# dv66/Distributed-Active-Learning

Measured on AMD Instinct MI355X. Metric: pool rows scored/sec (density-weighted uncertainty), 1–8 GPU; % MFMA/HBM peak, higher is better.
Workload: dtype f32 (fp16-split MFMA, fp32 accumulate); 1 GPU; config4: U[0,1) 2,000,000 x 256 fp32 pool (default_rng(0)), T=10 depth-4 forest, entropy x density, k=100, E={0..9}; pool_rows=2000000, features=256, trees=10, k=100, parallelism=single GPU

## Files before the change

### distributed-active-learning_amd/csrc/gram_csym_body.inc

```
  constexpr int HV = C::HALVES;
  __shared__ __attribute__((aligned(16))) float4 lds[2 * C::F4];
  __shared__ typename C::racc_t rowacc[HV * kSB];
  __shared__ int claim_lds[2];

  const int tid = threadIdx.x;
  const int wave = __builtin_amdgcn_readfirstlane(tid >> 6), lane = tid & 63;
  const int half = wave / C::WPS, wave4 = wave % C::WPS;
  if constexpr (C::WAVES == 8 && DAL_GRAM_PRIO8 != 0) {
    if (DAL_GRAM_PRIO8 > 0 ? wave >= 4 : wave < 4) __builtin_amdgcn_s_setprio(1);
  }
  const int li = lane & 15, lq = lane >> 4;
  const int G = gridDim.x, g = blockIdx.x;
  for (int e = tid; e < HV * kSB; e += C::NT) rowacc[e] = 0.0;

  const GramSchedule<HV> sched(srow0, n_srb, j_lo, j_hi, skip_lo, skip_hi, ns_active, chunk_j, n_chunks, contig, G,
                               g);

  constexpr int RPP = 64 / C::SLOTS;
  static_assert((RPP & (RPP - 1)) == 0 && (C::PIECES & (C::PIECES - 1)) == 0, "row parts must occupy disjoint bits");
  const unsigned rowbytes = static_cast<unsigned>(ldh * 2);
  const unsigned dst0 = __builtin_amdgcn_readfirstlane(
      static_cast<unsigned>(reinterpret_cast<uintptr_t>((AS3 float4*)(lds + wave * C::PIECES * 64))));
  auto issue = [&](int buf, int J, int h, int slice) {
    J = __builtin_amdgcn_readfirstlane(J);
    slice = __builtin_amdgcn_readfirstlane(slice);
    const char* sbase = reinterpret_cast<const char*>(
        ucols + (static_cast<int64_t>(J - jcol0) * 256 + h * C::SC) * ldh + slice_off + C::sub_off(slice));
    const unsigned fl = fresh_lane();
    const unsigned lrow = fl / C::SLOTS + static_cast<unsigned>(wave * C::PIECES * RPP);
    const unsigned vlane = lrow * rowbytes + (((fl % C::SLOTS) ^ static_cast<unsigned>(C::swz(lrow))) << 4);
#pragma unroll
    for (int q = 0; q < C::PIECES; ++q) {
      const unsigned dst = dst0 + static_cast<unsigned>(buf * C::STAGE + q * 1024);
      const unsigned voff = (vlane ^ (static_cast<unsigned>(C::swz(q * RPP)) << 4)) +
                            static_cast<unsigned>(q * RPP) * rowbytes;
      lds_dma_x4(voff, dst, sbase);
    }
  };

  f16x8 ah[C::RT][C::NKS];
  auto load_a = [&](int ru, int slice) {
    const int P = sched.rowP(ru, half);
    if (HV > 1 && !sched.live(P)) return;
    const uint16_t* pb = urows + static_cast<int64_t>(P - srow0) * kSB * ldh + slice_off + C::sub_off(slice);
    const unsigned fl = fresh_lane();
    const unsigned lrow = static_cast<unsigned>((wave4 * C::RPW + (fl & 15)) * ldh + (fl >> 4) * 8);
    const unsigned tstep = static_cast<unsigned>(16 * ldh);
#pragma unroll
    for (int rt = 0; rt < C::RT; ++rt)
#pragma unroll
      for (int c = 0; c < C::NKS; ++c)
        ah[rt][c] = __builtin_nontemporal_load(reinterpret_cast<const f16x8*>(pb + lrow + rt * tstep + c * C::LG * 8));
  };
  const int b_base = li * C::SLOTS + (lq ^ (C::swz(li) & 3));
  const int b_swz = C::swz(li) & ~3;
  auto b_off = [&](int c) { return b_base + ((c * C::LG) ^ b_swz); };

  typename C::acc4 mc[C::NCH][C::RT];
  [[maybe_unused]] const int mx_scale = kFp4ScaleWord;
  f16x8 bh[2];
  auto compute = [&](int buf, bool fresh_stage, int ct0 = 0, int ct1 = C::NCT) {
    auto load_b = [&](int set, int c, int ct) {
      bh[set] = __builtin_bit_cast(f16x8, lds[buf * C::F4 + ct * 16 * C::SLOTS + b_off(c)]);
    };
    if (ct0 == 0) load_b(0, 0, 0);
#pragma unroll
    for (int ct = ct0; ct < ct1; ++ct) {
      __builtin_amdgcn_sched_barrier(0);
      const bool fresh = fresh_stage && ct == 0;
#pragma unroll
      for (int c = 0; c < C::NKS; ++c) {
        constexpr int KPC = C::NKS / C::NCH;
        const int ch = c / KPC;
        const int i = ct * C::NKS + c, cur = i & 1;
        if (c + 1 < C::NKS)
          load_b(cur ^ 1, c + 1, ct);
        else if (ct + 1 < C::NCT)
          load_b(cur ^ 1, 0, ct + 1);
        const typename C::acc4 zero = {};
#pragma unroll
        for (int rt = 0; rt < C::RT; ++rt)
          mc[ch][rt] = C::mfma(bh[cur], ah[rt][c], (c % KPC == 0 && fresh) ? zero : mc[ch][rt], mx_scale);
      }
      constexpr int NM = C::RT;
#pragma unroll
      for (int c = 0; c < C::NKS; ++c) {
        __builtin_amdgcn_sched_group_barrier(0x100, 1, 0);
        __builtin_amdgcn_sched_group_barrier(0x008, NM, 0);
      }
      __builtin_amdgcn_sched_barrier(0);
    }
  };
  auto fold_rows = [&]() {
#pragma unroll
    for (int ch = 0; ch < C::NCH; ++ch)
#pragma unroll
      for (int t0 = 0; t0 < C::RT; t0 += 8) {
        typename C::sum_t x[8];
#pragma unroll
        for (int rt = 0; rt < 8; ++rt) {
          const typename C::acc4 m = mc[ch][t0 + rt];
          x[rt] = C::lane_sum(m);
        }
#pragma unroll
        for (int k = 0; k < 4; ++k) x[k] = swap_add<true>(x[k], x[k + 4]);
#pragma unroll
        for (int k = 0; k < 2; ++k) x[k] = swap_add<false>(x[k], x[k + 2]);
        const int row = wave * C::RPW + (t0 + 2 * (lq & 1) + 4 * (lq >> 1)) * 16 + li;
        C::row_add(&rowacc[row], x[0]);
        C::row_add(&rowacc[row + 16], x[1]);
      }
  };
  auto flush_one = [&](typename C::racc_t& slot, int64_t out_row) {
    const typename C::racc_t v = slot;
    if (v != 0) atomicAdd(acc_out + out_row, static_cast<unsigned long long>(static_cast<long long>(v)));
    slot = 0;
  };
  auto flush_rows = [&](int ru) {
    for (int e = tid; e < HV * kSB; e += C::NT) {
      const int P = sched.rowP(ru, e / kSB);
      if (sched.live(P)) flush_one(rowacc[e], static_cast<int64_t>(P) * kSB + e % kSB);
    }
  };
  auto block_sync = [&]() {
    asm volatile("s_waitcnt vmcnt(0) lgkmcnt(0)" ::: "memory");
    __syncthreads();
  };
  auto stage_sync = [&]() { block_sync(); };

  GramClaimCursor<HV> cur(sched, n_slices * C::NSUB);
  const bool dyn = claim_slot >= 0;
  int claim_par = 0;
  auto claim_begin = [&]() {
    if (dyn && tid == 0)
      claim_lds[claim_par] =
          G + static_cast<int>(__hip_atomic_fetch_add(&g_claim[claim_slot].next, 1u, __ATOMIC_RELAXED,
                                                      __HIP_MEMORY_SCOPE_AGENT));
  };
  auto claim_end = [&](int last) {
    const int u = dyn ? __builtin_amdgcn_readfirstlane(claim_lds[claim_par]) : cur.static_next(last);
    claim_par ^= 1;
    return u;
  };
  auto claim_take = [&]() {
    while (!cur.claimed(claim_end(cur.v_next))) {
      claim_begin();
      if (dyn) block_sync();
    }
  };
  auto leave = [&]() {
    if (dyn && tid == 0) {
      const unsigned before =
          __hip_atomic_fetch_add(&g_claim[claim_slot].done, 1u, __ATOMIC_RELAXED, __HIP_MEMORY_SCOPE_AGENT);
      if (before + 1 == static_cast<unsigned>(G)) {
        __hip_atomic_store(&g_claim[claim_slot].next, 0u, __ATOMIC_RELAXED, __HIP_MEMORY_SCOPE_AGENT);
        __hip_atomic_store(&g_claim[claim_slot].done, 0u, __ATOMIC_RELAXED, __HIP_MEMORY_SCOPE_AGENT);
      }
    }
  };
  if (!cur.claimed(cur.first_unit())) {
    claim_begin();
    if (dyn) block_sync();
    claim_take();
  }
  if (!cur.start()) {
    leave();
    return;
  }
  issue(0, cur.J, 0, cur.slice);
  load_a(cur.ru, cur.slice);
  claim_begin();
  int buf = 0;
  int flushRU = -1;

  while (true) {
    const bool act = cur.acts(half);

#pragma unroll
    for (int s = 0; s < C::SPP; ++s) {
      stage_sync();
      if constexpr (C::WIDE && DAL_GRAM_STAGGER > 0) {
        if (flushRU >= 0) {
          flush_rows(flushRU);
          flushRU = -1;
        }
        auto look_ahead = [&]() {
          if (cur.new_unit) claim_take();
          cur.peek();
          if (cur.has_next) issue(buf ^ 1, cur.next_J, 0, cur.next_slice());
        };
        const bool lead = lookahead_tiles(wave, C::WAVES, DAL_GRAM_STAGGER) == 0;
        if (!act) {
          look_ahead();
        } else {
          if (lead) look_ahead();
          compute(buf, true, 0, DAL_GRAM_STAGGER);
          if (!lead) look_ahead();
          compute(buf, true, DAL_GRAM_STAGGER, C::NCT);
          fold_rows();
        }
        buf ^= 1;
        continue;
      }
      if (s == 0) {
        if (cur.new_unit) claim_take();
        cur.peek();
        if (flushRU >= 0) {
          flush_rows(flushRU);
          flushRU = -1;
        }
      }
      if (s + 1 < C::SPP) {
        issue(buf ^ 1, cur.J, s + 1, cur.slice);
      } else if (cur.has_next) {
        issue(buf ^ 1, cur.next_J, 0, cur.next_slice());
      }
      if (act) {
        compute(buf, s % C::SPF == 0);
        if (s % C::SPF == C::SPF - 1) fold_rows();
      }
      buf ^= 1;
    }

    if (cur.rows_change) flushRU = cur.ru;
    if (!cur.has_next) break;
    if (cur.advance()) load_a(cur.ru, cur.slice);
    if (cur.new_unit) claim_begin();
  }
  block_sync();
  if (flushRU >= 0) flush_rows(flushRU);
  leave();
```

### distributed-active-learning_amd/csrc/gram_fp4.hpp

```cpp
#pragma once

#include "gram_i8.hpp"

#ifdef __HIPCC__
#define DAL_FP4_HD __host__ __device__
#else
#define DAL_FP4_HD
#endif

namespace dal {

constexpr float kFp4Step = 32.0f;
constexpr int kFp4AccShift = 18;
constexpr int kFp4Max = 12;
constexpr int kFp4ChainMax = 16 * 256 * kFp4Max * kFp4Max;
constexpr int kFp4RowMax = 256 * 256 * kFp4Max * kFp4Max;
static_assert(kFp4Step == kI8Step && kFp4AccShift == kI8AccShift, "the unit of G is the int8 form's");
static_assert(kFp4ChainMax == 589824 && 4 * kFp4ChainMax < (1 << 24),
              "fp32 chains and a lane's four columns are exact");
static_assert(kFp4RowMax == 9437184 && kFp4RowMax < (1LL << 31), "int32 row sums");

DAL_FP4_HD inline int quant_fp4(float h) {
  const float m = __builtin_fabsf(h) * (1.0f / kFp4Step);
  const int g = m > 10.0f ? 12 : m > 7.0f ? 8 : m > 5.0f ? 6 : m > 3.5f ? 4 : m > 2.5f ? 3 : m > 1.5f ? 2
                 : m > 0.5f ? 1 : 0;
  return h < 0.0f ? -g : g;
}

DAL_FP4_HD inline unsigned code_fp4(int g) {
  const unsigned m = static_cast<unsigned>(g < 0 ? -g : g);
  const unsigned idx = m <= 4u ? m : m == 6u ? 5u : m == 8u ? 6u : 7u;
  return idx | (g < 0 ? 8u : 0u);
}
DAL_FP4_HD inline int decode_fp4(unsigned code) {
  const unsigned idx = code & 7u;
  const int m = static_cast<int>(idx <= 4u ? idx : idx == 5u ? 6u : idx == 6u ? 8u : 12u);
  return code & 8u ? -m : m;
}

DAL_FP4_HD inline void requant_fp4(double& h, double& l) {
  const double hq = static_cast<double>(kFp4Step) * quant_fp4(static_cast<float>(h));
  l = (h - hq) + l;
  h = hq;
}

}
```

### distributed-active-learning_amd/csrc/gram_i8.hpp

```cpp
#pragma once

#ifdef __HIPCC__
#define DAL_I8_HD __host__ __device__
#else
#define DAL_I8_HD
#endif

namespace dal {

constexpr float kI8Step = 32.0f;
constexpr int kI8AccShift = 18;

DAL_I8_HD inline int quant_i8(float h) {
  const float q = __builtin_rintf(h * (1.0f / kI8Step));
  return static_cast<int>(q > 127.0f ? 127.0f : q >= -127.0f ? q : -127.0f);
}

DAL_I8_HD inline void requant_i8(double& h, double& l) {
  const double hq = static_cast<double>(kI8Step) * quant_i8(static_cast<float>(h));
  l = (h - hq) + l;
  h = hq;
}

}
```

### distributed-active-learning_amd/csrc/gram_schedule.hpp

```cpp
#pragma once

#include <stdint.h>

#include <utility>
#include <vector>

#if defined(__HIPCC__)
#define DAL_HD __host__ __device__ __forceinline__
#else
#define DAL_HD inline
#endif

namespace dal {

template <class I>
DAL_HD bool sb_takes(I P, I Q) {
  return Q == P || (Q > P && ((P + Q) & 1) == 0) || (Q < P && ((P + Q) & 1));
}

template <int HV>
struct GramSchedule {
  static_assert(HV == 1 || HV == 2 || HV == 4, "one, two or four super blocks per row unit");
  static constexpr bool form_ok(int contig) { return HV == 1 || !contig; }

  int srow0, n_srb, j_lo, j_hi, skip_lo, skip_hi, ns_active, chunk_j, n_chunks, contig, G, g;
  int n_ru;
  int sk_lo, skl;
  int nje;
  int nre;
  int64_t ka, kb;
  int n_seg;

  DAL_HD GramSchedule(int srow0_, int n_srb_, int j_lo_, int j_hi_, int skip_lo_, int skip_hi_, int ns_active_,
                      int chunk_j_, int n_chunks_, int contig_, int G_ = 1, int g_ = 0)
      : srow0(srow0_), n_srb(n_srb_), j_lo(j_lo_), j_hi(j_hi_), skip_lo(skip_lo_), skip_hi(skip_hi_),
        ns_active(ns_active_), chunk_j(chunk_j_), n_chunks(n_chunks_), contig(contig_), G(G_), g(g_) {
    n_ru = HV == 1 ? n_srb : 2 * ((n_srb + 2 * HV - 1) / (2 * HV));
    sk_lo = skip_lo > j_lo ? skip_lo : j_lo;
    const int sk_hi = skip_hi < j_hi ? skip_hi : j_hi;
    skl = contig && sk_hi > sk_lo ? sk_hi - sk_lo : 0;
    nje = j_hi - j_lo - skl;
    const int nre0 = ns_active - srow0;
    nre = nre0 < n_srb ? (nre0 > 0 ? nre0 : 0) : n_srb;
    ka = raw() * g / G;
    kb = raw() * (g + 1) / G;
    n_seg = contig ? (kb > ka ? static_cast<int>((kb - 1) / nje - ka / nje) + 1 : 0) : n_units();
  }

  DAL_HD int64_t raw() const { return static_cast<int64_t>(nre) * nje; }
  DAL_HD int n_units() const { return n_ru * n_chunks; }
  DAL_HD int first_seg() const { return contig ? 0 : g; }
  DAL_HD int seg_step() const { return contig ? 1 : G; }

  DAL_HD int rowP(int ru, int h) const {
    return HV == 1 ? srow0 + ru : srow0 + 2 * HV * (ru >> 1) + (ru & 1) + 2 * h;
  }
  DAL_HD bool live(int P) const { return P < srow0 + n_srb && P < ns_active; }
  DAL_HD int seg_ru(int u) const { return contig ? static_cast<int>(ka / nje) + u : u % n_ru; }
  DAL_HD int seg_rlo(int u) const {
    return contig ? (u == 0 ? static_cast<int>(ka % nje) : 0) : (u / n_ru) * chunk_j;
  }
  DAL_HD int seg_rhi(int u) const {
    if (contig) return u == n_seg - 1 ? static_cast<int>((kb - 1) % nje) + 1 : nje;
    const int e = (u / n_ru + 1) * chunk_j;
    return e < nje ? e : nje;
  }
  DAL_HD int jmap(int r) const { return j_lo + r + (j_lo + r >= sk_lo ? skl : 0); }
  DAL_HD bool takes(int P, int J) const {
    if (J >= skip_lo && J < skip_hi) return false;
    return sb_takes(P, J >> 1);
  }
  DAL_HD bool takes_h(int ru, int h, int J) const { return live(rowP(ru, h)) && takes(rowP(ru, h), J); }
  DAL_HD bool takes_u(int ru, int J) const {
    for (int h = 0; h < HV; ++h)
      if (takes_h(ru, h, J)) return true;
    return false;
  }
  DAL_HD int first_r(int ru, int r, int rhi) const {
    if constexpr (HV == 1) {
      const int P = srow0 + ru;
      if (P >= ns_active) return -1;
      while (r < rhi && !takes(P, jmap(r))) ++r;
    } else {
      if (!live(rowP(ru, 0))) return -1;
      const int P0 = rowP(ru, 0);
      while (r < rhi) {
        const int J = jmap(r), Q = J >> 1;
        if (skl == 0 && (Q < P0 || Q > P0 + 2 * HV - 2) && !(J >= skip_lo && J < skip_hi)) {
          if (((P0 + Q) & 1) == (Q < P0 ? 1 : 0)) break;
          r = 2 * (Q + 1) - j_lo;
          continue;
        }
        if (takes_u(ru, J)) break;
        ++r;
      }
    }
    return r < rhi ? r : -1;
  }
  DAL_HD int seek(int u, int& r) const {
    while (u < n_seg) {
      r = first_r(seg_ru(u), seg_rlo(u), seg_rhi(u));
      if (r >= 0) break;
      u += seg_step();
    }
    return u;
  }
};

template <int HV>
struct GramCursor {
  const GramSchedule<HV>& s;
  int unit = 0, r = -1, rhi_u = 0;
  int ru = -1, J = -1;
  int next_unit = 0, next_r = -1, next_ru = -1, next_J = -1;
  bool has_next = false, rows_change = false;

  DAL_HD explicit GramCursor(const GramSchedule<HV>& sched) : s(sched) {}
  DAL_HD bool start() {
    unit = s.seek(s.first_seg(), r);
    if (unit >= s.n_seg) return false;
    ru = s.seg_ru(unit);
    rhi_u = s.seg_rhi(unit);
    J = s.jmap(r);
    return true;
  }
  DAL_HD void peek() {
    next_r = s.first_r(ru, r + 1, rhi_u);
    next_unit = unit;
    if (next_r < 0) next_unit = s.seek(unit + s.seg_step(), next_r);
    has_next = next_unit < s.n_seg;
    next_ru = has_next ? s.seg_ru(next_unit) : -1;
    rows_change = next_ru != ru;
    next_J = has_next ? s.jmap(next_r) : -1;
  }
  DAL_HD bool advance() {
    unit = next_unit;
    rhi_u = s.seg_rhi(unit);
    ru = next_ru;
    r = next_r;
    J = next_J;
    return rows_change;
  }
  DAL_HD bool acts(int h) const { return HV == 1 || s.takes_h(ru, h, J); }
};

template <int HV>
struct GramClaimCursor {
  const GramSchedule<HV>& s;
  int n_slices;
  int v_next = -1, c_slice = -1, c_ru = -1, c_r = -1, c_rhi = 0;
  int slice = 0, ru = -1, r = -1, rhi_u = 0, J = -1;
  int next_r = -1, next_J = -1;
  bool has_next = false, rows_change = false, new_unit = false;

  DAL_HD GramClaimCursor(const GramSchedule<HV>& sched, int n_slices_)
      : s(sched), n_slices(sched.contig ? 1 : n_slices_) {}
  DAL_HD int total() const { return s.contig ? s.n_seg : n_slices * s.n_units(); }
  DAL_HD int first_unit() const { return s.first_seg(); }
  DAL_HD int static_next(int u) const { return u + s.seg_step(); }
  DAL_HD bool claimed(int u) {
    v_next = u;
    c_r = -1;
    if (u >= total()) return true;
    const int sg = s.contig ? u : u % s.n_units();
    c_slice = s.contig ? 0 : u / s.n_units();
    c_ru = s.seg_ru(sg);
    c_rhi = s.seg_rhi(sg);
    c_r = s.first_r(c_ru, s.seg_rlo(sg), c_rhi);
    return c_r >= 0;
  }
  DAL_HD bool start() {
    if (c_r < 0) return false;
    open();
    new_unit = true;
    return true;
  }
  DAL_HD int next_slice() const { return new_unit ? c_slice : slice; }
  DAL_HD int next_ru() const { return new_unit ? c_ru : ru; }
  DAL_HD void peek() {
    next_r = s.first_r(ru, r + 1, rhi_u);
    new_unit = next_r < 0;
    has_next = true;
    rows_change = false;
    if (new_unit) {
      has_next = c_r >= 0;
      next_r = c_r;
      rows_change = !has_next || c_ru != ru || c_slice != slice;
    }
    next_J = has_next ? s.jmap(next_r) : -1;
  }
  DAL_HD bool advance() {
    if (new_unit) {
      open();
    } else {
      r = next_r;
      J = next_J;
    }
    return rows_change;
  }
  DAL_HD bool acts(int h) const { return HV == 1 || s.takes_h(ru, h, J); }

 private:
  DAL_HD void open() {
    slice = c_slice;
    ru = c_ru;
    rhi_u = c_rhi;
    r = c_r;
    J = s.jmap(r);
  }
};

DAL_HD constexpr int lookahead_tiles(int wave, int waves, int stagger) { return wave < waves / 2 ? 0 : stagger; }


inline int64_t sb_pairs(int64_t I, int64_t lo, int64_t hi) {
  auto same_parity = [](int64_t a, int64_t b, int64_t p) -> int64_t {
    if (b <= a) return 0;
    return (b - p + 1) / 2 - (a - p + 1) / 2;
  };
  int64_t n = (lo <= I && I < hi) ? 1 : 0;
  n += same_parity(lo > I + 1 ? lo : I + 1, hi, I & 1);
  n += same_parity(lo, hi < I ? hi : I, (I & 1) ^ 1);
  return n;
}

inline int64_t pairs_range(int64_t P, int64_t a, int64_t b) {
  if (b <= a) return 0;
  const int64_t qa = a >> 1, qb = (b - 1) >> 1;
  int64_t n = 2 * sb_pairs(P, qa, qb + 1);
  if ((a & 1) && sb_takes(P, qa)) --n;
  if (!((b - 1) & 1) && sb_takes(P, qb)) --n;
  return n;
}
inline int64_t pairs_skip(int64_t P, int64_t a, int64_t b, int64_t skip_lo, int64_t skip_hi) {
  const int64_t sa = a > skip_lo ? a : skip_lo, sb = b < skip_hi ? b : skip_hi;
  return pairs_range(P, a, b) - pairs_range(P, sa, sb);
}

inline void column_chunks(int64_t nj, int64_t nc, int64_t* chunk_j, int64_t* n_chunks) {
  *chunk_j = (nj + nc - 1) / nc;
  *n_chunks = (nj + *chunk_j - 1) / *chunk_j;
}

template <int HV>
int64_t chunked_max_load(int64_t srow0, int64_t n_srb, int64_t lo, int64_t hi, int64_t skip_lo, int64_t skip_hi,
                         int64_t ns_active, int64_t G0, int64_t nc, int64_t* n_chunks) {
  int64_t cbk;
  column_chunks(hi - lo, nc, &cbk, n_chunks);
  auto sched = [&](int64_t G, int64_t g) {
    return GramSchedule<HV>(static_cast<int>(srow0), static_cast<int>(n_srb), static_cast<int>(lo),
                            static_cast<int>(hi), static_cast<int>(skip_lo), static_cast<int>(skip_hi),
                            static_cast<int>(ns_active), static_cast<int>(cbk), static_cast<int>(*n_chunks), 0,
                            static_cast<int>(G), static_cast<int>(g));
  };
  const int64_t units = sched(1, 0).n_units(), G = units < G0 ? units : G0;
  int64_t mx = 0;
  for (int64_t g = 0; g < G; ++g) {
    const GramSchedule<HV> s = sched(G, g);
    int64_t load = 0;
    for (int u = s.first_seg(); u < s.n_seg; u += s.seg_step()) {
      int64_t w = 0;
      for (int h = 0; h < HV; ++h) {
        const int P = s.rowP(s.seg_ru(u), h);
        if (!s.live(P)) continue;
        const int64_t pw = pairs_skip(P, lo + s.seg_rlo(u), lo + s.seg_rhi(u), skip_lo, skip_hi);
        w = pw > w ? pw : w;
      }
      load += w;
    }
    mx = load > mx ? load : mx;
  }
  return mx;
}

inline int64_t choose_chunks(int64_t srow0, int64_t n_srb, int64_t lo, int64_t hi, int64_t skip_lo, int64_t skip_hi,
                             int64_t ns_active, int64_t G0, int hv, int64_t kMinChunks) {
  struct Entry {
    int64_t k[10];
    int64_t nc;
  };
  static thread_local Entry cache[8] = {};
  static thread_local int cache_next = 0;
  const int64_t key[10] = {srow0, n_srb, lo, hi, skip_lo, skip_hi, ns_active, G0, hv, kMinChunks};
  for (const Entry& e : cache) {
    bool hit = e.nc > 0;
    for (int i = 0; i < 10 && hit; ++i) hit = e.k[i] == key[i];
    if (hit) return e.nc;
  }
  const int64_t nj = hi - lo;
  int64_t best_max = -1;
  std::vector<std::pair<int64_t, int64_t>> cand;
  int tried = 0;
  for (int64_t c = kMinChunks > 16 && nj >= kMinChunks ? kMinChunks : 1; c <= nj && tried < 32; ++c) {
    if (c > 1 && (nj + c - 1) / c == (nj + c - 2) / (c - 1)) continue;
    ++tried;
    int64_t ncc;
    const int64_t mx = hv == 1   ? chunked_max_load<1>(srow0, n_srb, lo, hi, skip_lo, skip_hi, ns_active, G0, c, &ncc)
                       : hv == 2 ? chunked_max_load<2>(srow0, n_srb, lo, hi, skip_lo, skip_hi, ns_active, G0, c, &ncc)
                                 : chunked_max_load<4>(srow0, n_srb, lo, hi, skip_lo, skip_hi, ns_active, G0, c, &ncc);
    cand.emplace_back(ncc, mx);
    if (best_max < 0 || mx < best_max) best_max = mx;
  }
  int64_t best_nc = -1;
  for (int pass = 0; pass < 2 && best_nc < 0; ++pass)
    for (const auto& c : cand)
      if ((pass || c.first >= kMinChunks) && c.second * 100 <= best_max * 108) {
        best_nc = c.first;
        break;
      }
  if (best_nc < 0) best_nc = cand.back().first;
  Entry& e = cache[cache_next];
  cache_next = (cache_next + 1) % 8;
  for (int i = 0; i < 10; ++i) e.k[i] = key[i];
  e.nc = best_nc;
  return best_nc;
}

struct GramLaunch {
  int chunk_j, n_chunks, G;
  int units;
};
template <int HV>
GramLaunch plan_launch(int64_t srow0, int64_t n_srb, int64_t j_lo, int64_t j_hi, int64_t skip_lo, int64_t skip_hi,
                       int64_t ns_active, int64_t G0, int contig, int64_t min_chunks, int64_t n_slices = 1) {
  int64_t cbk = j_hi - j_lo, n_chunks = 1;
  if (!contig)
    column_chunks(j_hi - j_lo,
                  choose_chunks(srow0, n_srb, j_lo, j_hi, skip_lo, skip_hi, ns_active, G0, HV, min_chunks), &cbk,
                  &n_chunks);
  const GramSchedule<HV> s(static_cast<int>(srow0), static_cast<int>(n_srb), static_cast<int>(j_lo),
                           static_cast<int>(j_hi), static_cast<int>(skip_lo), static_cast<int>(skip_hi),
                           static_cast<int>(ns_active), static_cast<int>(cbk), static_cast<int>(n_chunks), contig);
  const int64_t work = contig ? s.raw() : s.n_units() * n_slices;
  return {static_cast<int>(cbk), static_cast<int>(n_chunks), static_cast<int>(work < G0 ? (work > 0 ? work : 0) : G0),
          contig ? 0 : static_cast<int>(work)};
}

}
```

### distributed-active-learning_amd/csrc/gram_sym.hip

```cpp
#include <stdlib.h>

#include <mutex>
#include <type_traits>

#include "common.hpp"
#include "gram_fp4.hpp"
#include "gram_i8.hpp"
#include "gram_schedule.hpp"

namespace dal {
namespace {

typedef _Float16 f16x8 __attribute__((ext_vector_type(8)));
typedef float f32x4 __attribute__((ext_vector_type(4)));
typedef float f32x2 __attribute__((ext_vector_type(2)));
typedef int i32x4 __attribute__((ext_vector_type(4)));
typedef int i32x8 __attribute__((ext_vector_type(8)));
#define AS3 __attribute__((address_space(3)))

constexpr int kSB = 512;

__device__ __forceinline__ f32x4 mfma16(f16x8 a, f16x8 b, f32x4 c) {
  return __builtin_amdgcn_mfma_f32_16x16x32_f16(a, b, c, 0, 0, 0);
}

template <bool kRows32, typename T>
__device__ __forceinline__ T swap_add(T a, T b) {
  if constexpr (kRows32)
    asm volatile("s_nop 1\n\tv_permlane32_swap_b32 %0, %1" : "+v"(a), "+v"(b));
  else
    asm volatile("s_nop 1\n\tv_permlane16_swap_b32 %0, %1" : "+v"(a), "+v"(b));
  return a + b;
}

__device__ __forceinline__ unsigned fresh_lane() {
  unsigned v;
  asm volatile("v_mbcnt_lo_u32_b32 %0, -1, 0\n\tv_mbcnt_hi_u32_b32 %0, -1, %0" : "=v"(v));
  return v;
}

#ifndef DAL_GRAM_PRIO8
#define DAL_GRAM_PRIO8 1
#endif
#ifndef DAL_GRAM_KS64_OCC
#define DAL_GRAM_KS64_OCC 4
#endif
#ifndef DAL_GRAM_FOLD64
#define DAL_GRAM_FOLD64 256
#endif
#ifndef DAL_GRAM_FOLD128
#define DAL_GRAM_FOLD128 256
#endif
#ifndef DAL_GRAM_STAGE8
#define DAL_GRAM_STAGE8 32768
#endif
#ifndef DAL_GRAM_STAGGER
#define DAL_GRAM_STAGGER 4
#endif
#ifndef DAL_GRAM_CHAIN_MAX
#define DAL_GRAM_CHAIN_MAX 2048
#endif
#ifndef DAL_GRAM_W8_KS64
#define DAL_GRAM_W8_KS64 0
#endif
#ifndef DAL_GRAM_W8_OCC64
#define DAL_GRAM_W8_OCC64 1
#endif
#ifndef DAL_GRAM_KS32_OCC
#define DAL_GRAM_KS32_OCC 5
#endif
constexpr int kFormF16 = 0, kFormI8 = 1, kFormFp4 = 2;
constexpr int kFp4ScaleWord = static_cast<int>(0x80808080u);
template <int KS, int W = 4, int HVS = W / 4, int FORM = kFormF16>
struct Cfg {
  static constexpr bool I8 = FORM == kFormI8;
  static constexpr bool FP4 = FORM == kFormFp4;
  static constexpr bool INT = I8 || FP4;
  static constexpr int WAVES = W;
  static constexpr int HALVES = HVS;
  static constexpr bool WIDE = HVS == 4;
  static constexpr int KW = WIDE && !INT ? KS / 2 : KS;
  static constexpr int NSUB = KS / KW;
  static constexpr int WPS = W / HVS;
  static constexpr int RPW = kSB / WPS;
  static constexpr int NT = 64 * W;
  static constexpr int ROWB = FP4 ? KW / 2 : KW * (I8 ? 1 : 2);
  static constexpr int sub_off(int q) {
    return FP4 ? q * KS / 4 : I8 ? q * KS / 2 : (q / NSUB) * 2 * KS + (q % NSUB) * KW;
  }
  static constexpr int SLOTS = ROWB / 16;
  static constexpr int OCC = W == 8 ? (KS == 64 ? DAL_GRAM_W8_OCC64 : 1)
                                    : KS == 32 ? DAL_GRAM_KS32_OCC : KS == 64 ? DAL_GRAM_KS64_OCC : 2;
  static constexpr int STAGE = W == 8 ? DAL_GRAM_STAGE8 : OCC >= 4 ? 8192 : OCC == 3 ? 16384 : 32768;
  static constexpr int SC = STAGE / ROWB;
  static constexpr int SPP = 256 / SC;
  static_assert(SC >= 16 && SC <= 256, "a stage holds 16 to 256 whole columns");
  static constexpr int FOLD = KS >= 128 ? DAL_GRAM_FOLD128 : DAL_GRAM_FOLD64;
  static constexpr int SPF = FOLD / SC;
  static constexpr int F4 = STAGE / 16;
  static constexpr int SWZ = SLOTS - 1;
  static constexpr int swz(int row) {
    return SLOTS >= 8 ? row & SWZ : ((row >> 2) & 3) ^ (((row >> 2) & 1) << 1);
  }
  static_assert(SLOTS == 4 || SLOTS == 8 || SLOTS == 16, "swizzles for 4, 8 and 16 slots per row");
  static constexpr int PIECES = STAGE / (W * 1024);
  static constexpr int RT = RPW / 16;
  static constexpr int LG = 4;
  static constexpr int NKS = KW / (FP4 ? 128 : I8 ? 64 : 32);
  static constexpr int NCT = SC / 16;
  static constexpr int NCH = KW == 128 && !I8 ? 2 : 1;
  static constexpr int CHAIN = FOLD / 16 * (KW / NCH);
  static constexpr int CHARGED = KS == 32 ? DAL_GRAM_CHAIN_MAX / 2 : DAL_GRAM_CHAIN_MAX;
  static_assert(SPF >= 1 && SPP % SPF == 0 && PIECES >= 1 && NKS >= 1, "bad slice");
  static_assert(W == 4 || (W == 8 && KS >= 64), "several super blocks per block: KS >= 64 only");
  static_assert(!WIDE || (W == 8 && KS == (FP4 ? 256 : 128)), "the wide form: 8 waves at KS 128 (fp4: 256)");
  static_assert(FP4 == (KS == 256), "256-feature slices are the fp4 form's");
  static_assert(INT || (NKS % NCH == 0 && KW / NCH == 64 / (KS == 32 ? 2 : 1)),
                "a chain is 64 features of every tile (KS 32: 32)");
  static_assert(INT || CHAIN <= CHARGED, "row chain longer than the density bound charges");
  static_assert(!INT || (WIDE && ROWB == 128 && NSUB == 1 && NKS == 2 && NCH == 1),
                "the int8 and fp4 forms: the wide form over whole slices");
  static_assert(!I8 || FOLD <= 256, "int32 row chains: at most a pair's 256 columns between folds");
  static_assert(!FP4 || (FOLD / 16 * KW * kFp4Max * kFp4Max == kFp4ChainMax &&
                         FOLD * KW * kFp4Max * kFp4Max == kFp4RowMax),
                "fp32 chains of exact integers, int32 row sums");

  using acc4 = typename std::conditional<I8, i32x4, f32x4>::type;
  using sum_t = typename std::conditional<INT, int, float>::type;
  using racc_t = typename std::conditional<INT, long long, double>::type;
  static __device__ __forceinline__ acc4 mfma(f16x8 a, f16x8 b, acc4 c, [[maybe_unused]] int scale) {
    if constexpr (FP4) {
      const i32x4 a4 = __builtin_bit_cast(i32x4, a), b4 = __builtin_bit_cast(i32x4, b);
      const i32x8 a8 = {a4[0], a4[1], a4[2], a4[3], 0, 0, 0, 0}, b8 = {b4[0], b4[1], b4[2], b4[3], 0, 0, 0, 0};
      return __builtin_amdgcn_mfma_scale_f32_16x16x128_f8f6f4(a8, b8, c, 4, 4, 0, scale, 0, scale);
    } else if constexpr (I8) {
      return __builtin_amdgcn_mfma_i32_16x16x64_i8(__builtin_bit_cast(i32x4, a), __builtin_bit_cast(i32x4, b), c, 0,
                                                   0, 0);
    } else {
      return mfma16(a, b, c);
    }
  }
  static __device__ __forceinline__ sum_t lane_sum(acc4 m) {
    return static_cast<sum_t>((m[0] + m[1]) + (m[2] + m[3]));
  }
  static __device__ __forceinline__ void row_add(racc_t* slot, sum_t x) {
    if constexpr (INT)
      atomicAdd(reinterpret_cast<unsigned long long*>(slot),
                static_cast<unsigned long long>(static_cast<long long>(x) << kI8AccShift));
    else
      atomicAdd(slot, static_cast<double>(__builtin_rintf(x * 0x1p8f)));
  }
};
static_assert(Cfg<128, 8, 4>::CHAIN == Cfg<128, 4>::CHAIN, "the KS-128 forms define the same chains");

struct ClaimSlot {
  unsigned next, done;
};
constexpr int kClaimSlots = 64;
__device__ ClaimSlot g_claim[kClaimSlots];

template <int KS, int W, int HVS>
__global__ __launch_bounds__(64 * W, (Cfg<KS, W, HVS>::OCC)) void gram_csym_kernel(
    const uint16_t* __restrict__ urows, int srow0, int n_srb,
    const uint16_t* __restrict__ ucols, int jcol0, int j_lo, int j_hi, int skip_lo, int skip_hi,
    int ns_active, int64_t ldh, int slice_off, int n_slices, int chunk_j, int n_chunks,
    unsigned long long* __restrict__ acc_out, int contig, int claim_slot) {
  using C = Cfg<KS, W, HVS>;
#include "gram_csym_body.inc"
}
__global__ __launch_bounds__(512, 1) void gram_i8sym_kernel(
    const uint16_t* __restrict__ urows, int srow0, int n_srb,
    const uint16_t* __restrict__ ucols, int jcol0, int j_lo, int j_hi, int skip_lo, int skip_hi,
    int ns_active, int64_t ldh, int slice_off, int n_slices, int chunk_j, int n_chunks,
    unsigned long long* __restrict__ acc_out, int contig, int claim_slot) {
  using C = Cfg<128, 8, 4, kFormI8>;
#include "gram_csym_body.inc"
}
__global__ __launch_bounds__(512, 1) void gram_fp4sym_kernel(
    const uint16_t* __restrict__ urows, int srow0, int n_srb,
    const uint16_t* __restrict__ ucols, int jcol0, int j_lo, int j_hi, int skip_lo, int skip_hi,
    int ns_active, int64_t ldh, int slice_off, int n_slices, int chunk_j, int n_chunks,
    unsigned long long* __restrict__ acc_out, int contig, int claim_slot) {
  using C = Cfg<256, 8, 4, kFormFp4>;
#include "gram_csym_body.inc"
}

template <int kForm>
__device__ __forceinline__ void requant(double& h, double& l) {
  if constexpr (kForm == kFormFp4)
    requant_fp4(h, l);
  else
    requant_i8(h, l);
}
template <int kForm>
__global__ __launch_bounds__(256) void csym_sigma_kernel(const uint16_t* __restrict__ ops, int64_t ldh, int ks,
                                                         int d_pad, int ns, int qg, long long* __restrict__ sig_u,
                                                         long long* __restrict__ sl) {
  __shared__ long long red[256][9];
  const int cpr = static_cast<int>(ldh / 8);
  const int cols = cpr < 256 ? cpr : 256;
  const int col = blockIdx.y * 256 + threadIdx.x % cols;
  const int rstep = 256 / cols;
  const int r0 = threadIdx.x / cols;
  const int rb = kSB * static_cast<int>(blockIdx.z) / static_cast<int>(gridDim.z);
  const int re = kSB * (static_cast<int>(blockIdx.z) + 1) / static_cast<int>(gridDim.z);
  const int hpc = ks / 8;
  const int slice = col / (2 * hpc), within = col % (2 * hpc);
  const int f0 = slice * ks + (within % hpc) * 8;
  const bool l_col = within >= hpc;
  const bool finisher = threadIdx.x < cols && col < cpr;
  const int q_end = (static_cast<int>(blockIdx.x) + 1) * qg < ns ? (static_cast<int>(blockIdx.x) + 1) * qg : ns;
  long long lsum[8] = {};
  for (int Q = static_cast<int>(blockIdx.x) * qg; Q < q_end; ++Q) {
    double acc[8] = {};
    if (col < cpr && r0 < rstep) {
      const uint4* base = reinterpret_cast<const uint4*>(ops + static_cast<int64_t>(Q) * kSB * ldh) + col;
      for (int r = rb + r0; r < re; r += 8 * rstep) {
        uint4 q[8];
#pragma unroll
        for (int j = 0; j < 8; ++j)
          q[j] = r + j * rstep < re ? base[static_cast<int64_t>(r + j * rstep) * cpr] : uint4{};
        [[maybe_unused]] uint4 qh[8];
        if constexpr (kForm != kFormF16) {
#pragma unroll
          for (int j = 0; j < 8; ++j)
            qh[j] = l_col && r + j * rstep < re ? base[static_cast<int64_t>(r + j * rstep) * cpr - hpc] : uint4{};
        }
#pragma unroll
        for (int j = 0; j < 8; ++j) {
          const uint32_t w[4] = {q[j].x, q[j].y, q[j].z, q[j].w};
          if constexpr (kForm != kFormF16) {
            const uint32_t wh[4] = {qh[j].x, qh[j].y, qh[j].z, qh[j].w};
#pragma unroll
            for (int e = 0; e < 8; ++e) {
              const auto term = [e](const uint32_t* v) {
                const uint16_t b = static_cast<uint16_t>(e & 1 ? v[e >> 1] >> 16 : v[e >> 1] & 0xFFFFu);
                return static_cast<double>(static_cast<float>(__builtin_bit_cast(_Float16, b)));
              };
              double h = l_col ? term(wh) : term(w), l = l_col ? term(w) : 0.0;
              requant<kForm>(h, l);
              acc[e] += l_col ? l : h;
            }
            continue;
          }
#pragma unroll
          for (int e = 0; e < 4; ++e) {
            acc[2 * e] += static_cast<double>(
                static_cast<float>(__builtin_bit_cast(_Float16, static_cast<uint16_t>(w[e] & 0xFFFFu))));
            acc[2 * e + 1] += static_cast<double>(
                static_cast<float>(__builtin_bit_cast(_Float16, static_cast<uint16_t>(w[e] >> 16))));
          }
        }
      }
    }
    if (l_col) {
#pragma unroll
      for (int e = 0; e < 8; ++e) lsum[e] += static_cast<long long>(acc[e] * 16777216.0);
    }
    if (Q > static_cast<int>(blockIdx.x) * qg) __syncthreads();
#pragma unroll
    for (int e = 0; e < 8; ++e) red[threadIdx.x][e] = static_cast<long long>(acc[e] * 16777216.0);
    __syncthreads();
    if (finisher && !l_col) {
      long long v[8] = {};
      for (int p = 0; p < rstep; ++p)
#pragma unroll
        for (int e = 0; e < 8; ++e) v[e] += red[p * cols + threadIdx.x][e];
      long long* dst = sig_u + static_cast<int64_t>(Q) * d_pad + f0;
#pragma unroll
      for (int e = 0; e < 8; ++e)
        if (v[e] != 0) atomicAdd(reinterpret_cast<unsigned long long*>(dst + e), static_cast<unsigned long long>(v[e]));
    }
  }
  __syncthreads();
#pragma unroll
  for (int e = 0; e < 8; ++e) red[threadIdx.x][e] = lsum[e];
  __syncthreads();
  if (finisher && l_col) {
    long long v[8] = {};
    for (int p = 0; p < rstep; ++p)
#pragma unroll
      for (int e = 0; e < 8; ++e) v[e] += red[p * cols + threadIdx.x][e];
#pragma unroll
    for (int e = 0; e < 8; ++e)
      if (v[e] != 0) atomicAdd(reinterpret_cast<unsigned long long*>(sl + f0 + e), static_cast<unsigned long long>(v[e]));
  }
}

#ifndef DAL_CSYM_SCAN_WAVES
#define DAL_CSYM_SCAN_WAVES 16
#endif
constexpr int kScanWaves = DAL_CSYM_SCAN_WAVES;
constexpr int kScanBatch = 16;
#ifndef DAL_CSYM_FUSED_MAX
#define DAL_CSYM_FUSED_MAX 65536
#endif
__global__ __launch_bounds__(64 * kScanWaves) void csym_scan_kernel(const long long* __restrict__ sig_u, int ns,
                                                                    int d_pad, int b0, int b1, const long long* sl,
                                                                    double* st, double* __restrict__ cb) {
  constexpr int kW = kScanWaves;
  __shared__ long long part[kW][2][64];
  const int lane = threadIdx.x & 63, w = threadIdx.x >> 6;
  const int f = blockIdx.x * 64 + lane;
  const bool live = f < d_pad;
  const int q0 = static_cast<int>(static_cast<int64_t>(ns) * w / kW);
  const int q1 = static_cast<int>(static_cast<int64_t>(ns) * (w + 1) / kW);
  long long ue = 0, uo = 0;
  const long long s_l = live ? sl[f] : 0;
  if (live) {
    for (int qb = q0; qb < q1; qb += kScanBatch) {
      long long v[kScanBatch];
#pragma unroll
      for (int j = 0; j < kScanBatch; ++j)
        v[j] = qb + j < q1 ? sig_u[static_cast<int64_t>(qb + j) * d_pad + f] : 0;
#pragma unroll
      for (int j = 0; j < kScanBatch; ++j) {
        const bool odd = (qb + j) & 1;
        ue += odd ? 0 : v[j];
        uo += odd ? v[j] : 0;
      }
    }
  }
  part[w][0][lane] = ue;
  part[w][1][lane] = uo;
  __syncthreads();
  long long eue = 0, euo = 0, tue = 0, tuo = 0;
  for (int v = 0; v < kW; ++v) {
    const long long a0 = part[v][0][lane], a1 = part[v][1][lane];
    if (v < w) {
      eue += a0;
      euo += a1;
    }
    tue += a0;
    tuo += a1;
  }
  if (!live) return;
  if (w == 0) st[f] = static_cast<double>(tue + tuo + s_l);
  for (int qb = q0; qb < q1; qb += kScanBatch) {
    long long v[kScanBatch];
#pragma unroll
    for (int j = 0; j < kScanBatch; ++j)
      v[j] = qb + j < q1 ? sig_u[static_cast<int64_t>(qb + j) * d_pad + f] : 0;
#pragma unroll
    for (int j = 0; j < kScanBatch; ++j) {
      const int q = qb + j;
      const bool odd = q & 1;
      if (q < q1 && q >= b0 && q < b1) {
        const long long ch = odd ? (euo + tue - eue) : (eue + tuo - euo);
        cb[static_cast<int64_t>(q - b0) * d_pad + f] = static_cast<double>(ch + s_l);
      }
      eue += odd ? 0 : v[j];
      euo += odd ? v[j] : 0;
    }
  }
}

constexpr int kResRows = 256;
constexpr int kResFeat = 32;
constexpr int kResQ = kResFeat / 4;
constexpr int kResLd = kResQ + 1;
constexpr int kResStaged = 0, kResFused = 1, kResGlobal = 2;
constexpr int kResLdsMaxFeat = 1024;
template <int kMode, int kForm = kFormF16>
__global__ __launch_bounds__(kResRows) void csym_residual_kernel(const uint16_t* __restrict__ rows, int64_t ldh, int ks,
                                                                 int d_pad, int b0, int n_rows,
                                                                 const double* __restrict__ st,
                                                                 const double* __restrict__ cb,
                                                                 const long long* __restrict__ sig_u, int ns,
                                                                 long long* __restrict__ acc) {
  extern __shared__ double rc[];
  __shared__ uint4 tile[kResRows * kResLd];
  const int tid = threadIdx.x;
  const int64_t r0 = static_cast<int64_t>(blockIdx.x) * kResRows;
  const int64_t B = r0 / kSB;
  if constexpr (kMode == kResFused) {
    __shared__ long long red[8][kResRows];
    const int qB = b0 + static_cast<int>(B);
    const int hp = d_pad / 2, G = kResRows / hp, fp = tid % hp, grp = tid / hp;
    long long pe[2] = {}, po[2] = {}, te[2] = {}, to[2] = {};
    const longlong2* su2 = reinterpret_cast<const longlong2*>(sig_u);
    for (int qb = grp; qb < ns; qb += kScanBatch * G) {
      longlong2 v[kScanBatch];
#pragma unroll
      for (int j = 0; j < kScanBatch; ++j) {
        const int q = qb + j * G;
        v[j] = q < ns ? su2[static_cast<int64_t>(q) * hp + fp] : longlong2{0, 0};
      }
#pragma unroll
      for (int j = 0; j < kScanBatch; ++j) {
        const int q = qb + j * G;
        const bool odd = q & 1, before = q < qB;
#pragma unroll
        for (int c = 0; c < 2; ++c) {
          const long long x = c ? v[j].y : v[j].x;
          te[c] += odd ? 0 : x;
          to[c] += odd ? x : 0;
          pe[c] += before && !odd ? x : 0;
          po[c] += before && odd ? x : 0;
        }
      }
    }
#pragma unroll
    for (int c = 0; c < 2; ++c) {
      red[4 * c][tid] = pe[c];
      red[4 * c + 1][tid] = po[c];
      red[4 * c + 2][tid] = te[c];
      red[4 * c + 3][tid] = to[c];
    }
    __syncthreads();
    if (tid < hp) {
#pragma unroll
      for (int c = 0; c < 2; ++c) {
        long long eue = 0, euo = 0, tue = 0, tuo = 0;
        for (int g = 0; g < G; ++g) {
          eue += red[4 * c][g * hp + tid];
          euo += red[4 * c + 1][g * hp + tid];
          tue += red[4 * c + 2][g * hp + tid];
          tuo += red[4 * c + 3][g * hp + tid];
        }
        const bool odd = qB & 1;
        const int f = 2 * tid + c;
        const long long s_l = reinterpret_cast<const long long*>(st)[f];
        rc[f] = static_cast<double>(tue + tuo + s_l);
        rc[d_pad + f] = static_cast<double>((odd ? (euo + tue - eue) : (eue + tuo - euo)) + s_l);
      }
    }
  } else if constexpr (kMode == kResStaged) {
    for (int f = tid; f < d_pad; f += kResRows) {
      rc[f] = st[f];
      rc[d_pad + f] = cb[B * d_pad + f];
    }
  }
  const double* __restrict__ Sv = kMode == kResGlobal ? st : rc;
  const double* __restrict__ Dv = kMode == kResGlobal ? cb + B * d_pad : rc + d_pad;
  const int live_rows = n_rows - r0 < kResRows ? static_cast<int>(n_rows - r0) : kResRows;
  const uint16_t* blk = rows + r0 * ldh;
  double t = 0.0;
  for (int f0 = 0; f0 < d_pad; f0 += kResFeat) {
    const int64_t hoff = static_cast<int64_t>(f0 / ks) * 2 * ks + f0 % ks;
    uint4 q[kResQ];
#pragma unroll
    for (int j = 0; j < kResQ; ++j) {
      const int e = tid + kResRows * j;
      const int r = e / kResQ, c = e % kResQ;
      const int64_t off = r * ldh + hoff + (c < kResQ / 2 ? c * 8 : ks + (c - kResQ / 2) * 8);
      q[j] = r < live_rows ? *reinterpret_cast<const uint4*>(blk + off) : uint4{};
// ... 425 lines not shown
```

Baseline: 14.88 million rows/s.

## Defer row folds across several column pairs in integer gram forms

For the wide int8 and fp4 gram forms, MFMA accumulator chains are no longer zeroed and folded into LDS row sums after every pair. They now accumulate over up to FOLD_PAIRS pairs (7 for fp4, 3 for int8), with an early fold when the row block changes. Static asserts bound the pair count so fp32 chains stay exact integers and int32 row sums do not overflow. This cuts the per-pair lane reductions, swaps and LDS atomics, at the cost of recomputing lane indices to keep registers live across pairs. Whether it runs depends on whether config4 uses the fp4 or int8 path rather than f16.

```diff
diff --git a/distributed-active-learning_amd/csrc/gram_csym_body.inc b/distributed-active-learning_amd/csrc/gram_csym_body.inc
--- a/distributed-active-learning_amd/csrc/gram_csym_body.inc
+++ b/distributed-active-learning_amd/csrc/gram_csym_body.inc
@@ -57,11 +57,21 @@
   auto b_off = [&](int c) { return b_base + ((c * C::LG) ^ b_swz); };
 
   typename C::acc4 mc[C::NCH][C::RT];
+  constexpr bool kDefer = C::FOLD_PAIRS > 1;
   [[maybe_unused]] const int mx_scale = kFp4ScaleWord;
   f16x8 bh[2];
   auto compute = [&](int buf, bool fresh_stage, int ct0 = 0, int ct1 = C::NCT) {
+    [[maybe_unused]] int bb = 0, bs = 0;
+    if constexpr (kDefer) {
+      const int fl = static_cast<int>(fresh_lane()), fli = fl & 15, flq = fl >> 4;
+      bb = fli * C::SLOTS + (flq ^ (C::swz(fli) & 3));
+      bs = C::swz(fli) & ~3;
+    }
     auto load_b = [&](int set, int c, int ct) {
-      bh[set] = __builtin_bit_cast(f16x8, lds[buf * C::F4 + ct * 16 * C::SLOTS + b_off(c)]);
+      if constexpr (kDefer)
+        bh[set] = __builtin_bit_cast(f16x8, lds[buf * C::F4 + ct * 16 * C::SLOTS + bb + ((c * C::LG) ^ bs)]);
+      else
+        bh[set] = __builtin_bit_cast(f16x8, lds[buf * C::F4 + ct * 16 * C::SLOTS + b_off(c)]);
     };
     if (ct0 == 0) load_b(0, 0, 0);
 #pragma unroll
@@ -92,6 +102,12 @@
     }
   };
   auto fold_rows = [&]() {
+    [[maybe_unused]] int fli = 0, flq = 0;
+    if constexpr (kDefer) {
+      const int fl = static_cast<int>(fresh_lane());
+      fli = fl & 15;
+      flq = fl >> 4;
+    }
 #pragma unroll
     for (int ch = 0; ch < C::NCH; ++ch)
 #pragma unroll
@@ -106,11 +122,22 @@
         for (int k = 0; k < 4; ++k) x[k] = swap_add<true>(x[k], x[k + 4]);
 #pragma unroll
         for (int k = 0; k < 2; ++k) x[k] = swap_add<false>(x[k], x[k + 2]);
-        const int row = wave * C::RPW + (t0 + 2 * (lq & 1) + 4 * (lq >> 1)) * 16 + li;
+        const int row = kDefer ? wave * C::RPW + (t0 + 2 * (flq & 1) + 4 * (flq >> 1)) * 16 + fli
+                               : wave * C::RPW + (t0 + 2 * (lq & 1) + 4 * (lq >> 1)) * 16 + li;
         C::row_add(&rowacc[row], x[0]);
         C::row_add(&rowacc[row + 16], x[1]);
       }
   };
+  static_assert(!kDefer || (C::WIDE && C::SPP == 1 && DAL_GRAM_STAGGER > 0), "deferred folds: the wide form's pair loop");
+  [[maybe_unused]] int pending = 0;
+  [[maybe_unused]] auto zero_chains = [&]() {
+    const typename C::acc4 zero = {};
+#pragma unroll
+    for (int ch = 0; ch < C::NCH; ++ch)
+#pragma unroll
+      for (int rt = 0; rt < C::RT; ++rt) mc[ch][rt] = zero;
+  };
+  if constexpr (kDefer) zero_chains();
   auto flush_one = [&](typename C::racc_t& slot, int64_t out_row) {
     const typename C::racc_t v = slot;
     if (v != 0) atomicAdd(acc_out + out_row, static_cast<unsigned long long>(static_cast<long long>(v)));
@@ -194,10 +221,20 @@
           look_ahead();
         } else {
           if (lead) look_ahead();
-          compute(buf, true, 0, DAL_GRAM_STAGGER);
+          compute(buf, !kDefer, 0, DAL_GRAM_STAGGER);
           if (!lead) look_ahead();
-          compute(buf, true, DAL_GRAM_STAGGER, C::NCT);
-          fold_rows();
+          compute(buf, !kDefer, DAL_GRAM_STAGGER, C::NCT);
+          if constexpr (kDefer)
+            ++pending;
+          else
+            fold_rows();
+        }
+        if constexpr (kDefer) {
+          if (fold_due(pending, C::FOLD_PAIRS, cur.rows_change)) {
+            fold_rows();
+            zero_chains();
+            pending = 0;
+          }
         }
         buf ^= 1;
         continue;
diff --git a/distributed-active-learning_amd/csrc/gram_fp4.hpp b/distributed-active-learning_amd/csrc/gram_fp4.hpp
--- a/distributed-active-learning_amd/csrc/gram_fp4.hpp
+++ b/distributed-active-learning_amd/csrc/gram_fp4.hpp
@@ -19,6 +19,16 @@
 static_assert(kFp4ChainMax == 589824 && 4 * kFp4ChainMax < (1 << 24),
               "fp32 chains and a lane's four columns are exact");
 static_assert(kFp4RowMax == 9437184 && kFp4RowMax < (1LL << 31), "int32 row sums");
+constexpr long long kFp4ExactBelow = 1LL << 24;
+constexpr int kFp4FoldPairsMax = 7;
+constexpr int kFp4FoldPairsMaxEach = 28;
+static_assert(4LL * kFp4FoldPairsMax * kFp4ChainMax < kFp4ExactBelow &&
+                  4LL * (kFp4FoldPairsMax + 1) * kFp4ChainMax >= kFp4ExactBelow,
+              "a lane's fp32 sum of four chain elements over R pairs");
+static_assert(1LL * kFp4FoldPairsMaxEach * kFp4ChainMax < kFp4ExactBelow &&
+                  1LL * (kFp4FoldPairsMaxEach + 1) * kFp4ChainMax >= kFp4ExactBelow &&
+                  1LL * kFp4FoldPairsMaxEach * kFp4RowMax < (1LL << 31),
+              "one fp32 chain element over R pairs, and the int32 row sum");
 
 DAL_FP4_HD inline int quant_fp4(float h) {
   const float m = __builtin_fabsf(h) * (1.0f / kFp4Step);
diff --git a/distributed-active-learning_amd/csrc/gram_i8.hpp b/distributed-active-learning_amd/csrc/gram_i8.hpp
--- a/distributed-active-learning_amd/csrc/gram_i8.hpp
+++ b/distributed-active-learning_amd/csrc/gram_i8.hpp
@@ -11,6 +11,12 @@
 constexpr float kI8Step = 32.0f;
 constexpr int kI8AccShift = 18;
 
+constexpr long long kI8RowMax = 256LL * 128 * 128 * 128;
+constexpr int kI8FoldPairsMax = 3;
+static_assert(kI8RowMax == (1LL << 29) && kI8FoldPairsMax * kI8RowMax < (1LL << 31) &&
+                  (kI8FoldPairsMax + 1) * kI8RowMax >= (1LL << 31),
+              "int32 row sums over R pairs");
+
 DAL_I8_HD inline int quant_i8(float h) {
   const float q = __builtin_rintf(h * (1.0f / kI8Step));
   return static_cast<int>(q > 127.0f ? 127.0f : q >= -127.0f ? q : -127.0f);
diff --git a/distributed-active-learning_amd/csrc/gram_schedule.hpp b/distributed-active-learning_amd/csrc/gram_schedule.hpp
--- a/distributed-active-learning_amd/csrc/gram_schedule.hpp
+++ b/distributed-active-learning_amd/csrc/gram_schedule.hpp
@@ -211,6 +211,10 @@
 };
 
 DAL_HD constexpr int lookahead_tiles(int wave, int waves, int stagger) { return wave < waves / 2 ? 0 : stagger; }
+
+DAL_HD constexpr bool fold_due(int pending, int cap, bool rows_change) {
+  return pending >= cap || (pending > 0 && rows_change);
+}
 
 
 inline int64_t sb_pairs(int64_t I, int64_t lo, int64_t hi) {
diff --git a/distributed-active-learning_amd/csrc/gram_sym.hip b/distributed-active-learning_amd/csrc/gram_sym.hip
--- a/distributed-active-learning_amd/csrc/gram_sym.hip
+++ b/distributed-active-learning_amd/csrc/gram_sym.hip
@@ -56,6 +56,15 @@
 #endif
 #ifndef DAL_GRAM_STAGGER
 #define DAL_GRAM_STAGGER 4
+#endif
+#ifndef DAL_GRAM_FOLD_PAIRS_FP4
+#define DAL_GRAM_FOLD_PAIRS_FP4 7
+#endif
+#ifndef DAL_GRAM_FOLD_PAIRS_I8
+#define DAL_GRAM_FOLD_PAIRS_I8 3
+#endif
+#ifndef DAL_GRAM_FP4_CVT_EACH
+#define DAL_GRAM_FP4_CVT_EACH 0
 #endif
 #ifndef DAL_GRAM_CHAIN_MAX
 #define DAL_GRAM_CHAIN_MAX 2048
@@ -124,6 +133,13 @@
   static_assert(!FP4 || (FOLD / 16 * KW * kFp4Max * kFp4Max == kFp4ChainMax &&
                          FOLD * KW * kFp4Max * kFp4Max == kFp4RowMax),
                 "fp32 chains of exact integers, int32 row sums");
+  static constexpr bool CVT_EACH = FP4 && DAL_GRAM_FP4_CVT_EACH != 0;
+  static constexpr int FOLD_PAIRS = FP4 ? DAL_GRAM_FOLD_PAIRS_FP4 : I8 ? DAL_GRAM_FOLD_PAIRS_I8 : 1;
+  static_assert(FOLD_PAIRS >= 1 && (FOLD_PAIRS == 1 || (WIDE && FOLD == 256)),
+                "chains over several pairs: the wide integer forms, one fold group per pair");
+  static_assert(!I8 || FOLD_PAIRS <= kI8FoldPairsMax, "int32 row sums over FOLD_PAIRS pairs");
+  static_assert(!FP4 || FOLD_PAIRS <= (CVT_EACH ? kFp4FoldPairsMaxEach : kFp4FoldPairsMax),
+                "fp32 chains (and a lane's fp32 sum of four) of exact integers over FOLD_PAIRS pairs");
 
   using acc4 = typename std::conditional<I8, i32x4, f32x4>::type;
   using sum_t = typename std::conditional<INT, int, float>::type;
@@ -141,7 +157,10 @@
     }
   }
   static __device__ __forceinline__ sum_t lane_sum(acc4 m) {
-    return static_cast<sum_t>((m[0] + m[1]) + (m[2] + m[3]));
+    if constexpr (CVT_EACH)
+      return (static_cast<int>(m[0]) + static_cast<int>(m[1])) + (static_cast<int>(m[2]) + static_cast<int>(m[3]));
+    else
+      return static_cast<sum_t>((m[0] + m[1]) + (m[2] + m[3]));
   }
   static __device__ __forceinline__ void row_add(racc_t* slot, sum_t x) {
     if constexpr (INT)
```

After: 15.11 million rows/s (median of 6 runs). 1.6% higher.
